# craabreu/EmDee.jl

Hardware: AMD Instinct MI355X
Metric: md_steps_per_sec (higher is better)
Workload: dtype f64

## Files before the change

emdee.jl_amd/csrc/brick.hpp:

```cpp
#pragma once

#include "kernels.hpp"

namespace emdee {

enum BrickMode { BRICK_FORCE = 1, BRICK_STATS = 2, BRICK_STEP = 3 };

#define EMDEE_PLAIN_LOOP _Pragma("clang loop unroll(disable) vectorize(disable) interleave(disable)")

constexpr int EPL = 8;
constexpr int brick_prefetch_blocks(int G, int THREADS) { return (EPL * G) >= 128 ? 1 : ((G == 4 && THREADS >= 1024) ? 5 : 2); }
constexpr int brick_min_stride(int G, int THREADS) { return (brick_prefetch_blocks(G, THREADS) + 1) * EPL * G; }

template <int BX_, int BY_, int BZ_>
struct BrickShape {
    static constexpr int BX = BX_, BY = BY_, BZ = BZ_;
    static constexpr int TX = BX + 2, TY = BY + 2, TZ = BZ + 2;
    static constexpr int NTC = TX * TY * TZ;
    static constexpr int NOC = BX * BY * BZ;
};

struct BrickGrid {
    int nb[3];
    int nbricks;
// ... 1143 lines not shown
    auto slot = [&](unsigned short ent) {
        const int sl = (int)ent >> a.idx_shift;
        int lo = 0, hi = Shape::NTC;
        while (hi - lo > 1) {
            const int mid = (lo + hi) >> 1;
            if (T.off[mid] <= sl) lo = mid; else hi = mid;
        }
        return T.gbeg[lo] + (sl - T.off[lo]);
    };
    for (int o = threadIdx.x; o < n_own; o += THREADS) {
        int ti, p;
        brick_locate(T, o, ti, p);
        if (a.perm[p] >= a.n_owned) continue;
        const int m = min(a.cnt[p], a.stride);
        unsigned short *row = a.nbr + (size_t)p * a.stride;
        const int w = strike_row(keys, bk, a.perm, ex_start, ex_idx, p, m,
                                 [&](int e) -> unsigned short & { return row[row_position<G>((unsigned)e)]; }, slot);
        if (w < 0) continue;
        for (int e = w; e < m; e++) row[row_position<G>((unsigned)e)] = 0;
        a.cnt[p] = w;
    }
}

template <class Shape>
__global__ void k_brick_tile_max(BrickGrid bg, int Mx, int My, int Mz, int px, int py, int pz,
                                 const int *__restrict__ start, int *__restrict__ out) {
    const int b = blockIdx.x * blockDim.x + threadIdx.x;
    int total = 0, own = 0, span3 = 0;
    if (b < bg.nbricks) {
        const int bxi = b % bg.nb[0], byi = (b / bg.nb[0]) % bg.nb[1], bzi = b / (bg.nb[0] * bg.nb[1]);
        const int ox0 = bxi * Shape::BX, oy0 = byi * Shape::BY, oz0 = bzi * Shape::BZ;
        const int ox1 = min(ox0 + Shape::BX, Mx), oy1 = min(oy0 + Shape::BY, My), oz1 = min(oz0 + Shape::BZ, Mz);
        for (int tz = 0; tz < Shape::TZ; tz++)
            for (int ty = 0; ty < Shape::TY; ty++) {
                const int ry = oy0 - 1 + ty, rz = oz0 - 1 + tz;
                int gy = ry, gz = rz;
                if (gy > oy1 || gz > oz1) continue;
                if (gy < 0) { if (!py) continue; gy += My; } else if (gy >= My) { if (!py) continue; gy -= My; }
                if (gz < 0) { if (!pz) continue; gz += Mz; } else if (gz >= Mz) { if (!pz) continue; gz -= Mz; }
                int p1 = 0, p2 = 0;
                for (int tx = 0; tx < Shape::TX; tx++) {
                    const int rx = ox0 - 1 + tx;
                    int gx = rx;
                    bool valid = gx <= ox1;
                    if (gx < 0) { if (!px) valid = false; gx += Mx; } else if (gx >= Mx) { if (!px) valid = false; gx -= Mx; }
                    int pop = 0;
                    if (valid) {
                        const int c = gx + Mx * (gy + My * gz);
                        pop = start[c + 1] - start[c];
                        total += pop;
                        if (rx >= ox0 && rx < ox1 && ry >= oy0 && ry < oy1 && rz >= oz0 && rz < oz1) own += pop;
                    }
                    span3 = max(span3, pop + p1 + p2);
                    p2 = p1; p1 = pop;
                }
            }
    }
#pragma unroll
    for (int off = 1; off < WAVE; off <<= 1) {
        total = max(total, __shfl_xor(total, off));
        own = max(own, __shfl_xor(own, off));
        span3 = max(span3, __shfl_xor(span3, off));
    }
    if ((threadIdx.x & (WAVE - 1)) == 0 && total > 0) {
        atomicMax(&out[0], total);
        atomicMax(&out[1], own);
        atomicMax(&out[2], span3);
    }
}

}
```

emdee.jl_amd/csrc/kernels.hpp:

```cpp
#pragma once

#include <hip/hip_runtime.h>

#include "common.hpp"
#include "lj_pair.hpp"
#include "wave_ops.hpp"

namespace emdee {

template <typename real>
struct Rec;
template <>
struct alignas(32) Rec<double> {
    double x, y, z;
    float hs, te;
};
template <>
struct alignas(16) Rec<float> {
    float x, y, z, hs;
};

struct RelGrid {
    double lo[3], cw[3];
    int M[3];
// ... 217 lines not shown
        } else {
            cell_of[i] = -1;
        }
    }
    int first, len;
    wave_run(c, first, len);
    if (c >= 0 && lane_id() == first) atomicAdd(&count[c], len);
}

static __global__ void k_cell_scatter(int n, const int *__restrict__ cell_of, int one_based, const int *__restrict__ start,
                               int *__restrict__ fill, int *__restrict__ tmp) {
    int i = blockIdx.x * blockDim.x + threadIdx.x;
    const int c = (i < n) ? cell_of[i] - one_based : -1;
    int first, len;
    wave_run(c, first, len);
    int base = 0;
    if (c >= 0 && lane_id() == first) base = start[c] + atomicAdd(&fill[c], len);
    base = __shfl(base, first);
    if (c >= 0) tmp[base + (lane_id() - first)] = i;
}

static __global__ void k_cell_scatter_keyed(int n, const int *__restrict__ cell_of, const int *__restrict__ start,
                                            int *__restrict__ fill, const int *__restrict__ key, int2 *__restrict__ tmp,
                                            const long long *__restrict__ tag = nullptr) {
    int i = blockIdx.x * blockDim.x + threadIdx.x;
    const int c = (i < n) ? cell_of[i] : -1;
    int first, len;
    wave_run(c, first, len);
    int base = 0;
    if (c >= 0 && lane_id() == first) base = start[c] + atomicAdd(&fill[c], len);
    base = __shfl(base, first);
    if (c >= 0) tmp[base + (lane_id() - first)] = make_int2(i, tag ? (int)tag[i] : (key ? key[i] : i));
}
static __global__ void k_cell_rankfix_keyed(int n, const int *__restrict__ cell_of, const int *__restrict__ start,
                                            const int2 *__restrict__ tmp, int *__restrict__ order,
                                            const int *__restrict__ n_dev = nullptr, int ties = 1) {
    int q = blockIdx.x * blockDim.x + threadIdx.x;
    if (n_dev) n = min(n, *n_dev);
    if (q >= n) return;
    const int2 me = tmp[q];
    const int c = cell_of[me.x];
    const int s = start[c], e = start[c + 1];
    int rank = 0;
    if (ties) {
        for (int r = s; r < e; r++) {
            const int2 o = tmp[r];
            rank += (o.y < me.y || (o.y == me.y && o.x < me.x)) ? 1 : 0;
        }
    } else {
        for (int r = s; r < e; r++) rank += (tmp[r].y < me.y) ? 1 : 0;
    }
    order[s + rank] = me.x;
}

static __global__ void k_cell_rankfix(int n, const int *__restrict__ cell_of, int one_based, const int *__restrict__ start,
                               const int *__restrict__ tmp, const int *__restrict__ key, int *__restrict__ order) {
    int q = blockIdx.x * blockDim.x + threadIdx.x;
    if (q >= n) return;
    int i = tmp[q];
    int c = cell_of[i] - one_based;
    int s = start[c], e = start[c + 1];
    int ki = key ? key[i] : i;
    int rank = 0;
    for (int r = s; r < e; r++) {
        int j = tmp[r];
        int kj = key ? key[j] : j;
        rank += (kj < ki) ? 1 : 0;
    }
    order[s + rank] = i;
}

constexpr int SCAN_THREADS = 256;
constexpr int SCAN_ITEMS = 8;
constexpr int SCAN_TILE = SCAN_THREADS * SCAN_ITEMS;

// ... 125 lines not shown
constexpr int IMG_BIAS = 512;
__device__ __forceinline__ int img_pack(int kx, int ky, int kz) {
    return (kx + IMG_BIAS) | ((ky + IMG_BIAS) << 10) | ((kz + IMG_BIAS) << 20);
}
__device__ __forceinline__ void img_unpack(int v, int &kx, int &ky, int &kz) {
    kx = (v & 1023) - IMG_BIAS; ky = ((v >> 10) & 1023) - IMG_BIAS; kz = ((v >> 20) & 1023) - IMG_BIAS;
}
template <typename real>
__device__ __forceinline__ int wrap_into_box(real &p, real lo, real len, int periodic) {
    if (!periodic) return 0;
    const real k = floor((p - lo) / len);
    p -= k * len;
    return (int)k;
}

__device__ __forceinline__ int rel_nearest_image(double &r, double len, int periodic) {
    if (!periodic) return 0;
    const double s = rint(r / len);
    r -= s * len;
    return (int)s;
}

template <typename real>
__global__ void k_gather_user(int n, int n_owned, size_t pitch, GridP<real> g, const int *__restrict__ order,
                              const int *__restrict__ cell_of, const real *__restrict__ pos,
                              const emdee_lj_atom *__restrict__ atoms, const real *__restrict__ vel,
                              const real *__restrict__ inv_mass, Rec<real> *__restrict__ rec, float *__restrict__ te,
                              real *__restrict__ xb, real *__restrict__ v_out, real *__restrict__ im_out,
                              int *__restrict__ perm, int *__restrict__ inv_perm, int *__restrict__ cell_sorted,
                              int *__restrict__ img, int nt = 1, const long long *__restrict__ tag_in = nullptr,
                              long long *__restrict__ tag_out = nullptr, int ncell = 0, int *__restrict__ cstart = nullptr,
                              const int *__restrict__ tstart = nullptr, RelGrid rel_out = RelGrid{}) {
    int p = blockIdx.x * blockDim.x + threadIdx.x;
    if (cstart) for (int c = p; c <= ncell; c += gridDim.x * blockDim.x) cstart[c] = tstart[(size_t)c * nt];
    if (p >= n) return;
    int i = order[p];
    if (tag_out) tag_out[p] = tag_in[i];
    real x = pos[3 * (size_t)i], y = pos[3 * (size_t)i + 1], z = pos[3 * (size_t)i + 2];
    const int kx = wrap_into_box(x, g.lo[0], g.len[0], g.per[0]);
    const int ky = wrap_into_box(y, g.lo[1], g.len[1], g.per[1]);
    const int kz = wrap_into_box(z, g.lo[2], g.len[2], g.per[2]);
    img[p] = img_pack(kx, ky, kz);
    emdee_lj_atom a = atoms[i];
    if (sizeof(real) == 4 && rel_out.on) {
        double ox, oy, oz;
        rel_out.origin(cell_of[i] / nt, ox, oy, oz);
        double rx = (double)x - ox, ry = (double)y - oy, rz = (double)z - oz;
        int jx = kx + rel_nearest_image(rx, (double)g.len[0], g.per[0]), jy = ky + rel_nearest_image(ry, (double)g.len[1], g.per[1]),
            jz = kz + rel_nearest_image(rz, (double)g.len[2], g.per[2]);
        img[p] = img_pack(jx, jy, jz);
        x = (real)rx; y = (real)ry; z = (real)rz;
    }
    store_rec<real>(rec, te, p, x, y, z, a.half_sigma, a.twice_sqrt_eps);
    xb[p] = x; xb[pitch + p] = y; xb[2 * pitch + p] = z;
    bool owned = i < n_owned;
    if (v_out) {
        for (int d = 0; d < 3; d++) v_out[d * pitch + p] = (owned && vel) ? vel[3 * (size_t)i + d] : (real)0;
    }
    if (im_out) im_out[p] = (owned && inv_mass) ? inv_mass[i] : (real)1;
    perm[p] = i;
    inv_perm[i] = p;
    cell_sorted[p] = cell_of[i] / nt;
}

template <typename real, bool EDIT = false>
__global__ void k_gather_sorted(int n, size_t pitch, GridP<real> g, const int *__restrict__ order,
                                const int *__restrict__ cell_of, const Rec<real> *__restrict__ rec_in,
                                const float *__restrict__ te_in, const real *__restrict__ v_in,
                                const real *__restrict__ im_in, const int *__restrict__ perm_in,
                                const int *__restrict__ img_in, Rec<real> *__restrict__ rec, float *__restrict__ te,
                                real *__restrict__ xb, real *__restrict__ v_out, real *__restrict__ im_out,
                                int *__restrict__ perm, int *__restrict__ inv_perm, int *__restrict__ cell_sorted,
                                int *__restrict__ img, int nt = 1, const long long *__restrict__ tag_in = nullptr,
                                long long *__restrict__ tag_out = nullptr, const int *__restrict__ n_dev = nullptr,
                                int *__restrict__ n_out = nullptr, int ncell = 0, int *__restrict__ cstart = nullptr,
                                const int *__restrict__ tstart = nullptr, RelGrid rel_in = RelGrid{}, RelGrid rel_out = RelGrid{}) {
    int p = blockIdx.x * blockDim.x + threadIdx.x;
    if (cstart) for (int c = p; c <= ncell; c += gridDim.x * blockDim.x) cstart[c] = tstart[(size_t)c * nt];
    if (EDIT) {
        n = min(n, *n_dev);
        if (p == 0 && n_out) *n_out = *n_dev;
    }
    if (p >= n) return;
    int o = order[p];
    Rec<real> r = rec_in[o];
    float hs, tev;
    rec_params(rec_in, te_in, o, hs, tev);
    int kx = 0, ky = 0, kz = 0;
    if (!EDIT) img_unpack(img_in[o], kx, ky, kz);
    if (sizeof(real) == 4 && (rel_in.on || rel_out.on)) {
        double ax = (double)r.x, ay = (double)r.y, az = (double)r.z, ox, oy, oz;
        if (rel_in.on) { rel_in.origin(rel_in.cell[o], ox, oy, oz); ax += ox; ay += oy; az += oz; }
        kx += wrap_into_box(ax, (double)g.lo[0], (double)g.len[0], g.per[0]);
        ky += wrap_into_box(ay, (double)g.lo[1], (double)g.len[1], g.per[1]);
        kz += wrap_into_box(az, (double)g.lo[2], (double)g.len[2], g.per[2]);
        if (rel_out.on) {
            rel_out.origin(cell_of[o] / nt, ox, oy, oz); ax -= ox; ay -= oy; az -= oz;
            kx += rel_nearest_image(ax, (double)g.len[0], g.per[0]);
            ky += rel_nearest_image(ay, (double)g.len[1], g.per[1]);
            kz += rel_nearest_image(az, (double)g.len[2], g.per[2]);
        }
        r.x = (real)ax; r.y = (real)ay; r.z = (real)az;
    } else {
        kx += wrap_into_box(r.x, g.lo[0], g.len[0], g.per[0]);
        ky += wrap_into_box(r.y, g.lo[1], g.len[1], g.per[1]);
        kz += wrap_into_box(r.z, g.lo[2], g.len[2], g.per[2]);
    }
    img[p] = img_pack(kx, ky, kz);
    store_rec<real>(rec, te, p, r.x, r.y, r.z, hs, tev);
    xb[p] = r.x; xb[pitch + p] = r.y; xb[2 * pitch + p] = r.z;
    if (v_out) {
        for (int d = 0; d < 3; d++) v_out[d * pitch + p] = v_in[d * pitch + o];
    }
    if (im_out) im_out[p] = im_in[o];
    if (tag_out) tag_out[p] = tag_in[o];
    int i = EDIT ? o : perm_in[o];
    perm[p] = i;
    inv_perm[i] = p;
    cell_sorted[p] = cell_of[o] / nt;
}

template <typename real>
__global__ void k_refresh_positions(int n, size_t pitch, GridP<real> g, const int *__restrict__ perm,
                                    const real *__restrict__ pos, const emdee_lj_atom *__restrict__ atoms,
                                    const real *__restrict__ xb, Rec<real> *__restrict__ rec, float *__restrict__ te) {
    int p = blockIdx.x * blockDim.x + threadIdx.x;
    if (p >= n) return;
    int i = perm[p];
    emdee_lj_atom a = atoms[i];
    const real bx = xb[p], by = xb[pitch + p], bz = xb[2 * pitch + p];
    const real x = bx + min_image(pos[3 * (size_t)i] - bx, g.plen[0], g.pinv[0]);
    const real y = by + min_image(pos[3 * (size_t)i + 1] - by, g.plen[1], g.pinv[1]);
    const real z = bz + min_image(pos[3 * (size_t)i + 2] - bz, g.plen[2], g.pinv[2]);
    store_rec<real>(rec, te, p, x, y, z, a.half_sigma, a.twice_sqrt_eps);
}

template <typename real>
__global__ void k_refresh_check(int n, size_t pitch, GridP<real> g, const int *__restrict__ perm, const real *__restrict__ pos,
                                const emdee_lj_atom *__restrict__ atoms, const real *__restrict__ xb, Rec<real> *__restrict__ rec,
                                float *__restrict__ te, real thr2, int *__restrict__ flags, int typed = 0) {
    int p = blockIdx.x * blockDim.x + threadIdx.x;
    if (p >= n) return;
// ... 946 lines not shown
```

emdee.jl_amd/csrc/nbsys.hpp:

```cpp
#pragma once
#include <cstdio>

#include <algorithm>
#include <cmath>
#include <cstdlib>
#include <type_traits>

#include "brick.hpp"
#include "ewald.hpp"
#include "kernels.hpp"
#include "topology_dev.hpp"
#include "typed.hpp"

namespace emdee {

static inline void refuse_experiment_switches() {
    static const char *const gone[] = {"EMDEE_DEBUG_RC2_SCALE", "EMDEE_TBUILD", "EMDEE_BUILD4", "EMDEE_BUILD_ALG", "EMDEE_BUILD_CHUNKED",
        "EMDEE_BUILD_STRIDED", "EMDEE_NO_BRICK_TABLES", "EMDEE_NO_PREMUL", "EMDEE_BUILD_NEARFAR", "EMDEE_NEAR_DELTA", "EMDEE_FAR_SKIP",
        "EMDEE_PLAN_MAXIMA", "EMDEE_PLAN_SYNC", "EMDEE_STRIDE", "EMDEE_BRICK_VARIANT"};
    for (const char *name : gone)
        EMDEE_REQUIRE(std::getenv(name) == nullptr, EMDEE_ERR_INVALID,
                      "%s is an experiment switch that has been retired with the laboratory (make EXPERIMENTS=1 no longer "
                      "exists): the variant it selected is not built; its measurement is recorded in DESIGN.md, "
                      "\"Product and laboratory\"", name);
// ... 69 lines not shown
    GridP<real> grid{};
    size_t ncell = 0;
    int n_total = 0, n_owned = 0;
    size_t pitch = 0;
    bool with_vel = false, with_mass = false;
    bool sorted = false, has_list = false;
    int stride = 0;
    int64_t builds = 0;
    bool profiling = false;
    KernelTimer timers[T_COUNT];

    int path = PATH_BRICK;
    int variant = 0;
    BrickGrid bgrid{};
    int tile_cap = 0, own_cap = 0, row_block = 1;
    int build_alg = 1;
    bool field16_blocked = false;
    size_t lds_bytes = 0, lds_build_bytes = 0;
    float build_margin = 0.f;

    DevBuf<Rec<real>> rec, rec2;
    DevBuf<float> te, te2;
    DevBuf<real> vel, vel2, frc, en, vir, im, im2, xb, noise;
    DevBuf<int> perm, perm2, inv_perm, cell_of, cell_sorted, cell_sorted2, order, count, fill, nbr, cnt, flags, img, img2;
    DevBuf<int2> tmp2;
    DevBuf<long long> tag, tag2;
    bool use_tags = false;
    size_t cap_hint = 0;
    size_t capacity = 0;
    bool has_ghosts = false;
    int id_space = 0;
    bool id_gaps = false;
    DevBuf<int> cmap;
    bool cmap_valid = false;
    SpeciesTable species{1, {0, 0, 0, 0}};
    int nt = 1;
    int nsub = 1;
    bool subbins_enabled = std::getenv("EMDEE_NO_SUBBINS") == nullptr;
    int tsub = 1;
    bool typed_subbins_enabled = std::getenv("EMDEE_TYPED_SUBBINS") == nullptr || std::atoi(std::getenv("EMDEE_TYPED_SUBBINS")) != 0;
    int digits() const { return nt > 1 ? nt * tsub : nsub; }
    DevBuf<int> bsub;
    bool typed_enabled = std::getenv("EMDEE_NO_TYPED") == nullptr;
    DevBuf<int> cstart;
    DevBuf<unsigned long long> species_tab;
    DevBuf<unsigned short> nbr16;
    DevBuf<int> btab;
// ... 95 lines not shown
            g.per[d] = per[d];
            g.M[d] = M[d];
            cells *= (size_t)M[d];
        }
        g.nd = 1;
        g.one_based = 0;
        grid = g;
        ncell = cells;
    }

    void reserve(int n, bool velocities, bool masses) {
        n_total = n;
        const size_t m = std::max((size_t)n, cap_hint);
        capacity = m;
        pitch = (m + 63) / 64 * 64 + 64;
        with_vel = velocities;
        with_mass = masses;
        rec.ensure(m + 1); rec2.ensure(m + 1);
        if (sizeof(real) == 4) { te.ensure(m + 1); te2.ensure(m + 1); }
        frc.ensure(3 * pitch); en.ensure(pitch); vir.ensure(pitch); xb.ensure(3 * pitch);
        if (velocities) { vel.ensure(3 * pitch); vel2.ensure(3 * pitch); }
        if (masses) { im.ensure(pitch); im2.ensure(pitch); }
        perm.ensure(m + 1); perm2.ensure(m + 1); inv_perm.ensure(m + 1); img.ensure(m + 1); img2.ensure(m + 1);
        cell_of.ensure(m + 1); cell_sorted.ensure(m + 1); cell_sorted2.ensure(m + 1); order.ensure(m + 1); cnt.ensure(m + 1);
        if (use_tags) { tag.ensure(m + 1); tag2.ensure(m + 1); }
        if (flags.ensure(32)) EMDEE_HIP_CHECK(hipMemsetAsync(flags.ptr, 0, 32 * sizeof(int), stream()));
        partial.ensure(3 * RED_MAX_BLOCKS); sums.ensure(8); stats.ensure(4);
    }

    template <class Src, class Spc>
    void bin(Src src, const int *key, Spc spc, int n_items = -1, const long long *tagkey = nullptr, const unsigned char *keep = nullptr) {
        const int n = n_items >= 0 ? n_items : n_total;
        const int dm = digits();
        const size_t nbins = ncell * (size_t)dm;
        count.ensure(nbins + 2); fill.ensure(nbins + 2);
        Zeros zr;
        zr.add(count.ptr, nbins + 1).add(fill.ptr, nbins);
        if (dm > 1) {
            cstart.ensure(ncell + 2);
            if (n == 0) zr.add(cstart.ptr, ncell + 1);
        }
        zr.run(stream());
        if (n == 0) return;
        hipLaunchKernelGGL((k_cell_assign<real, Src, Spc>), dim3(blocks_for(n, 256)), dim3(256), 0, stream(), n, src, grid,
                           cell_of.ptr, count.ptr, spc, dm, keep);
        scanner.run(count.ptr, nbins + 1, stream());
        tmp2.ensure(std::max((size_t)n, capacity) + 1);
        hipLaunchKernelGGL(k_cell_scatter_keyed, dim3(blocks_for(n, 256)), dim3(256), 0, stream(), n, cell_of.ptr, count.ptr,
                           fill.ptr, key, tmp2.ptr, tagkey);
        hipLaunchKernelGGL(k_cell_rankfix_keyed, dim3(blocks_for(n, 256)), dim3(256), 0, stream(), n, cell_of.ptr, count.ptr,
                           tmp2.ptr, order.ptr, keep ? count.ptr + nbins : nullptr, tagkey != nullptr ? 1 : 0);
    }
    int sub_k() const {
        const double cx = len[0] / std::max(1, grid.M[0]);
        const double margin = 16.0 * grid.M[0] * (sizeof(real) == 4 ? 6.0e-8 : 1.2e-16) + 1e-9;
        return std::max(-1, (int)std::floor(4.0 * (1.0 - rlist * (1.0 + margin) / cx)));
    }
    void choose_subbins() {
        nsub = (subbins_enabled && path == PATH_BRICK && nt == 1 && n_total > 0) ? 4 : 1;
        tsub = (subbins_enabled && typed_subbins_enabled && typed_enabled && path == PATH_BRICK && nt == 2 && n_total > 0) ? 4 : 1;
    }
    template <class Src, class Spc>
    void bin_species(Src src, const int *key, Spc spc, int n_items = -1, const long long *tagkey = nullptr, const unsigned char *keep = nullptr) {
        using Sub = XSubBin<real, Src>;
        if (tsub > 1) bin(src, key, SpeciesSub<Spc, Sub>{spc, Sub{src, grid.lo[0], grid.len[0], grid.M[0], grid.per[0], tsub}}, n_items, tagkey, keep);
        else bin(src, key, spc, n_items, tagkey, keep);
    }
    template <class Src>
    void bin_untyped(Src src, const int *key, int n_items = -1, const long long *tagkey = nullptr, const unsigned char *keep = nullptr) {
        if (nsub > 1) bin(src, key, XSubBin<real, Src>{src, grid.lo[0], grid.len[0], grid.M[0], grid.per[0], nsub}, n_items, tagkey, keep);
        else bin(src, key, NoSpecies{}, n_items, tagkey, keep);
    }
    const int *start() const { return digits() > 1 ? cstart.ptr : count.ptr; }
    const int *tstart() const { return count.ptr; }

    void load_user(int n_own, int n_ghost, const real *pos, const real *velocities, const emdee_lj_atom *atoms,
                   const real *inv_mass, const long long *tags_user = nullptr) {
        EMDEE_REQUIRE(n_own >= 0 && n_ghost >= 0, EMDEE_ERR_INVALID, "negative atom count");
        EMDEE_REQUIRE((int64_t)n_own + n_ghost < (int64_t)1 << 31, EMDEE_ERR_INVALID, "too many atoms");
        EMDEE_REQUIRE(n_own + n_ghost == 0 || (pos && atoms), EMDEE_ERR_INVALID, "positions/atoms are NULL");
        Timed t(this, T_REBUILD);
        n_owned = n_own;
        has_ghosts = n_ghost > 0;
        id_space = n_own + n_ghost; id_gaps = false; cmap_valid = false;
        lgv_ids = nullptr;
        use_tags = tags_user != nullptr;
        reserve(n_own + n_ghost, velocities != nullptr || with_vel, inv_mass != nullptr);
        detect_uniform_atoms(atoms);
        configure_grid();
        const int n = n_total;
        const bool rel_next = rel_wanted();
        choose_subbins();
        if (nt > 1) bin_species(UserPos<real>{pos}, nullptr, UserSpecies{species, atoms}, -1, use_tags ? tags_user : nullptr);
        else bin_untyped(UserPos<real>{pos}, nullptr, -1, use_tags ? tags_user : nullptr);
        if (n > 0)
            hipLaunchKernelGGL((k_gather_user<real>), dim3(blocks_for(n, 256)), dim3(256), 0, stream(), n, n_owned, pitch,
                               grid, order.ptr, cell_of.ptr, pos, atoms, velocities, inv_mass, rec.ptr, te.ptr, xb.ptr,
                               with_vel ? vel.ptr : nullptr, with_mass ? im.ptr : nullptr, perm.ptr, inv_perm.ptr,
                               cell_sorted.ptr, img.ptr, digits(), use_tags ? tags_user : nullptr, use_tags ? tag.ptr : nullptr,
                               (int)ncell, digits() > 1 ? cstart.ptr : nullptr, count.ptr, rel_grid_next(rel_next, nullptr));
        rel_commit(rel_next);
        q_valid = false;
        if (has_ghosts)
            hipLaunchKernelGGL((k_copy_ghost_records<real>), dim3(blocks_for(n, 256)), dim3(256), 0, stream(), n, n_owned,
                               perm.ptr, rec.ptr, rec2.ptr);
        sorted = true;
        build_list();
    }

    void resort() {
        EMDEE_REQUIRE(sorted, EMDEE_ERR_STATE, "no state loaded");
        Timed t(this, T_REBUILD);
        const int n = n_total;
        configure_grid();
        choose_subbins();
        const long long *tk = use_tags ? tag.ptr : nullptr;
        const RelGrid rel_in = rel_grid(rel_now, cell_sorted.ptr);
        const bool rel_next = rel_wanted();
        if (nt > 1) bin_species(RecPos<real>{rec.ptr, rel_in}, perm.ptr, RecSpecies<real>{species, rec.ptr, te.ptr}, -1, tk);
        else bin_untyped(RecPos<real>{rec.ptr, rel_in}, perm.ptr, -1, tk);
        if (n > 0)
            hipLaunchKernelGGL((k_gather_sorted<real, false>), dim3(blocks_for(n, 256)), dim3(256), 0, stream(), n, pitch, grid,
                               order.ptr, cell_of.ptr, rec.ptr, te.ptr, with_vel ? vel.ptr : nullptr,
                               with_mass ? im.ptr : nullptr, perm.ptr, img.ptr, rec2.ptr, te2.ptr, xb.ptr,
                               with_vel ? vel2.ptr : nullptr, with_mass ? im2.ptr : nullptr, perm2.ptr, inv_perm.ptr,
                               cell_sorted2.ptr, img2.ptr, digits(), tk, use_tags ? tag2.ptr : nullptr, (const int *)nullptr,
                               (int *)nullptr, (int)ncell, digits() > 1 ? cstart.ptr : nullptr, count.ptr, rel_in,
                               rel_grid_next(rel_next, nullptr));
        swap_sorted_buffers();
        rel_commit(rel_next);
        build_list();
    }
    void check_scaled_box(const double mu[3], double vscale) const {
        for (int d = 0; d < 3; d++)
            EMDEE_REQUIRE(std::isfinite(mu[d]) && mu[d] > 0.0, EMDEE_ERR_INVALID, "scale_box: mu[%d] = %g must be finite and > 0", d, mu[d]);
        EMDEE_REQUIRE(std::isfinite(vscale) && vscale > 0.0, EMDEE_ERR_INVALID, "scale_box: velocity_scale = %g must be finite and > 0", vscale);
        for (int d = 0; d < 3; d++) {
            const double nl = mu[d] * len[d];
            EMDEE_REQUIRE(std::isfinite(nl) && nl > 0.0, EMDEE_ERR_INVALID, "scale_box: the new box length %g along %d is not finite and > 0", nl, d);
            EMDEE_REQUIRE(!per[d] || nl >= 2.0 * rlist, EMDEE_ERR_INVALID, "scale_box: the new periodic box length %g along dimension %d is below "
                          "2 (cutoff + skin) = %g (minimum image)", nl, d, 2.0 * rlist);
        }
    }
    void scale_box(const double mu[3], double vscale) {
        EMDEE_REQUIRE(sorted && with_vel && !has_ghosts, EMDEE_ERR_STATE, "scale_box: needs a loaded state without ghosts");
        check_scaled_box(mu, vscale);
        if (n_total > 0) {
            ScaleBox s{};
            for (int d = 0; d < 3; d++) { s.lo[d] = lo[d]; s.mu[d] = mu[d]; }
            hipLaunchKernelGGL((k_cell_state_scale<real>), dim3(blocks_for(n_total, 256)), dim3(256), 0, stream(), n_total, pitch, rec.ptr,
                               vel.ptr, s, (real)vscale, vscale != 1.0 ? 1 : 0, rel_grid(rel_now, cell_sorted.ptr));
// ... 13 lines not shown

    struct EditWords {
        const int *dev = nullptr;
        int n = 0;
        int32_t *host = nullptr;
    };
    bool in_edit = false, edit_abort = false;
    EditWords edit_extra{};
    int edit_n_plan = 0;
    struct EditSaved { int n_total, n_owned, id_space; bool id_gaps, has_ghosts, has_list; } edit_saved{};
    bool edit_fits(int n_items) const { return sorted && use_tags && with_vel && !with_mass && (size_t)n_items <= capacity; }
    bool edit_extra_read = false;
    bool resort_edit(int n_items, const unsigned char *keep, int own_limit, bool ghosts, int *n_live_dev, EditWords extra) {
        EMDEE_REQUIRE(edit_fits(n_items), EMDEE_ERR_STATE, "resort_edit: the state does not hold %d slots", n_items);
        Timed t(this, T_REBUILD);
        edit_saved = EditSaved{n_total, n_owned, id_space, id_gaps, has_ghosts, has_list};
        configure_grid();
        choose_subbins();
        EMDEE_REQUIRE(!rel_now, EMDEE_ERR_STATE, "resort_edit: cell-relative records (decomposed domains keep absolute ones)");
        if (nt > 1) bin_species(RecPos<real>{rec.ptr, RelGrid{}}, nullptr, RecSpecies<real>{species, rec.ptr, te.ptr}, n_items, tag.ptr, keep);
        else bin_untyped(RecPos<real>{rec.ptr, RelGrid{}}, nullptr, n_items, tag.ptr, keep);
        const size_t nbins = ncell * (size_t)digits();
        hipLaunchKernelGGL((k_gather_sorted<real, true>), dim3(blocks_for(n_items, 256)), dim3(256), 0, stream(), n_items, pitch, grid,
                           order.ptr, cell_of.ptr, rec.ptr, te.ptr, vel.ptr, (const real *)nullptr, perm.ptr, img.ptr, rec2.ptr, te2.ptr,
                           xb.ptr, vel2.ptr, (real *)nullptr, perm2.ptr, inv_perm.ptr, cell_sorted2.ptr, img2.ptr, digits(), tag.ptr,
                           tag2.ptr, count.ptr + nbins, n_live_dev, (int)ncell, digits() > 1 ? cstart.ptr : nullptr, count.ptr);
        swap_sorted_buffers();
        edit_n_plan = n_total;
        n_total = n_items;
        n_owned = own_limit;
        has_ghosts = ghosts;
        id_space = n_items; id_gaps = true; cmap_valid = false;
        in_edit = true; edit_abort = false; edit_extra = extra; edit_extra_read = false;
        struct Leave { bool &f; ~Leave() { f = false; } } leave{in_edit};
        if (path == PATH_BRICK && plan_valid && edit_saved.n_total > 0) build_list();
        else edit_abort = true;
        if (edit_abort && !edit_extra_read && extra.n > 0) read_back_words(ctx, stream(), extra.dev, extra.n, extra.host);
        return !edit_abort;
    }
    void commit_edit(int n_live) {
        EMDEE_REQUIRE(n_live >= 0 && n_live <= n_total, EMDEE_ERR_STATE, "resort_edit: %d atoms in %d slots", n_live, n_total);
        n_total = n_live;
        if (has_ghosts && n_total > 0)
            hipLaunchKernelGGL((k_copy_ghost_records<real>), dim3(blocks_for(n_total, 256)), dim3(256), 0, stream(), n_total, n_owned,
                               perm.ptr, rec.ptr, rec2.ptr);
    }
    void rollback_edit() {
        swap_sorted_buffers();
        n_total = edit_saved.n_total; n_owned = edit_saved.n_owned; id_space = edit_saved.id_space;
// ... 147 lines not shown
            bgrid.nbricks = bgrid.nb[0] * bgrid.nb[1] * bgrid.nb[2];
            bgrid.per_xcd = (bgrid.nbricks + NXCD - 1) / NXCD;
            const int B[3] = {S::BX, S::BY, S::BZ};
            bgrid.ib_count = 1;
            for (int d = 0; d < 3; d++) {
                int lo_b = 0, n_b = bgrid.nb[d];
                if (!grid.per[d]) {
                    lo_b = 1;
                    int hi_b = 1;
                    while (hi_b < bgrid.nb[d] && (hi_b + 1) * B[d] < grid.M[d] - 1) hi_b++;
                    n_b = std::max(0, hi_b - lo_b);
                }
                bgrid.ib_lo[d] = lo_b; bgrid.ib_n[d] = n_b;
                bgrid.ib_count *= n_b;
            }
            bgrid.ib_per_xcd = (bgrid.ib_count + NXCD - 1) / NXCD;
            bgrid.bb_z = (bgrid.nb[2] - bgrid.ib_n[2]) * bgrid.nb[0] * bgrid.nb[1];
            bgrid.bb_y = bgrid.ib_n[2] * (bgrid.nb[1] - bgrid.ib_n[1]) * bgrid.nb[0];
            bgrid.bb_count = bgrid.nbricks - bgrid.ib_count;
            bgrid.bb_per_xcd = (bgrid.bb_count + NXCD - 1) / NXCD;
            row_block = EPL * V::G;
        });
    }
    void launch_tile_max(bool with_build_words = false) {
        with_brick_variant(variant, [&](auto v) {
            using S = typename decltype(v)::Shape;
            if (with_build_words) Zeros().add(flags.ptr, 9).run(stream());
            else Zeros().add(flags.ptr + 6, 3).run(stream());
            hipLaunchKernelGGL((k_brick_tile_max<S>), dim3(blocks_for(bgrid.nbricks, 256)), dim3(256), 0, stream(), bgrid,
                               grid.M[0], grid.M[1], grid.M[2], grid.per[0], grid.per[1], grid.per[2], start(),
                               flags.ptr + 6);
        });
    }
    static int with_headroom(int v) { return (v + v / 32 + 8 + 15) / 16 * 16; }
    bool plan_sizes(int max_tile, int max_own, int max_span3) {
        bool ok = true;
        with_brick_variant(variant, [&](auto v) {
            using V = decltype(v);
            using S = typename V::Shape;
            tile_cap = std::max(64, with_headroom(max_tile + 1));
            if (max_tile + 1 <= SOA_SLOTS) tile_cap = std::min(tile_cap, SOA_SLOTS);
            own_cap = std::max(64, with_headroom(max_own));
            {
                const int exact = std::max(64, (max_tile + 1 + 15) / 16 * 16), st = stride > 0 ? stride : 128;
                constexpr size_t USABLE = 150000;
                auto per_cu = [&](int tc) {
                    const size_t b = brick_build_lds_bytes<S, V::THREADS>(tc, own_cap, st, V::GB, nsub),
                                 f = brick_force_lds_bytes<real, S, V::THREADS>(tc, own_cap, has_charges());
                    return (int)(USABLE / std::max<size_t>(b, 1)) * 16 + (int)(USABLE / std::max<size_t>(f, 1));
                };
                while (tile_cap > exact && per_cu(tile_cap) < per_cu(exact)) tile_cap -= 16;
            }
// ... 140 lines not shown
    bool typed_blocked = false;
    bool typed_stride = false;

    void build_list() {
        const int n = n_total;
        if (stride == 0) {
            double vol = len[0] * len[1] * len[2];
            double expect = n > 0 ? (4.0 / 3.0) * M_PI * rlist * rlist * rlist * (double)n / vol : 0.0;
            stride = (int)((expect * 1.15 + 8.0) / 16.0 + 1.0) * 16;
            typed_stride = false;
        }
        btab_valid = false;
        const int np = in_edit ? edit_n_plan : n;
        bool kept = plan_valid && path == PATH_BRICK && n > 0 && plan_M[0] == grid.M[0] &&
                    plan_M[1] == grid.M[1] && plan_M[2] == grid.M[2] && plan_n <= np + np / 8 && np <= plan_n + plan_n / 8 &&
                    plan_uniform == uniform_atoms && plan_nt == nt && plan_charged == has_charges();
        if (kept) {
            plan_geometry();
            launch_tile_max(true);
            brick_active = true;
        } else {
            make_plan();
        }
        const size_t rows = std::max<size_t>((size_t)std::max(n, 1), cap_hint ? capacity : 0);
        for (int attempt = 0; attempt < 6; attempt++) {
            EMDEE_REQUIRE((double)n * stride < 1.7e10, EMDEE_ERR_OVERFLOW, "neighbour list would exceed 64 GiB");
            if (in_edit && !brick_active) { edit_abort = true; return; }
            if (!(kept && attempt == 0)) Zeros().add(flags.ptr, 5).run(stream());
            if (brick_active) {
                nbr16.ensure(rows * stride);
                with_brick_variant(variant, [&](auto v) {
                    using V = decltype(v);
                    if constexpr (typed_variant<V>()) {
                        if (typed_active) {
                            constexpr int TT = 256;
                            using BT = TypedTables<typename V::Shape, TT>;
                            static_assert(BT::row_ints() == TypedTables<typename V::Shape, V::THREADS>::row_ints(), "table row layout");
                            btab.ensure((size_t)bgrid.nbricks * BT::row_ints());
                            BrickArgs<real> ta = brick_args();
                            ta.btab = btab.ptr;
                            if (tsub > 1) {
                                bsub.ensure((size_t)bgrid.nbricks * BT::NTT + 4);
                                ta.nsub = tsub; ta.bsub = bsub.ptr;
                            }
                            hipLaunchKernelGGL((k_typed_tables<real, typename V::Shape, TT>), dim3(bgrid.per_xcd * NXCD), dim3(TT),
                                               BT::bytes(0), stream(), ta);
// ... 375 lines not shown
        if (has_post()) return false;
        if (phase != 2 && !noise_ready) prepare_noise(dt);
        {
            Timed t(this, phase == 2 ? T_STEP_BOUNDARY : T_STEP);
            step_c = c; step_dt = dt;
            force_phase = phase;
            step_guard = guard; step_trigger = trigger;
            with_brick_variant(variant, [&](auto v) { launch_brick_kernel<decltype(v), BRICK_STEP, 1>(); });
            step_guard = nullptr; step_trigger = nullptr;
        }
        if (phase != 1 && lgv_on) lgv_step++;
        if (phase != 1) {
            if (carry_ghosts && has_ghosts)
                hipLaunchKernelGGL((k_copy_ghost_records<real>), dim3(blocks_for(n_total, 256)), dim3(256), 0, stream(),
                                   n_total, n_owned, perm.ptr, rec.ptr, rec2.ptr);
            swap_step_buffers();
        }
        return true;
    }
    void swap_step_buffers() { rec.swap(rec2); vel.swap(vel2); }

    static constexpr int RUN_AHEAD = 4;
    int run_ahead = RUN_AHEAD;
    int *step_trigger = nullptr;
    const int *step_guard = nullptr;
    int fused_steps_run_ahead(double c, double dt, int want, bool *stale) {
        EMDEE_REQUIRE(has_list && sorted && with_vel, EMDEE_ERR_STATE, "no state loaded");
        *stale = false;
        if (!brick_active || n_total == 0 || has_ghosts || has_post()) return 0;
        const int B = std::max(1, std::min(want, run_ahead));
        int *words = flags.ptr + 9;
        EMDEE_HIP_CHECK(hipMemsetAsync(words, 0, B * sizeof(int), stream()));
        step_c = c; step_dt = dt; force_phase = 0;
        for (int i = 0; i < B; i++) {
            prepare_noise(dt);
            if (lgv_on) lgv_step++;
            Timed t(this, T_STEP);
            step_trigger = words + i;
            step_guard = i ? words + i - 1 : nullptr;
            with_brick_variant(variant, [&](auto v) { launch_brick_kernel<decltype(v), BRICK_STEP, 1>(); });
            swap_step_buffers();
        }
        step_trigger = nullptr; step_guard = nullptr;
        read_back_words(ctx, stream(), words, B, ctx->host_flags + 9);
        int ran = B;
        for (int i = 0; i < B; i++)
            if (ctx->host_flags[9 + i]) { ran = i + 1; *stale = true; break; }
        if ((B - ran) & 1) swap_step_buffers();
        if (lgv_on) lgv_step -= (unsigned long long)(B - ran);
        if (profiling) timers[T_STEP].dropped += B - ran;
        return ran;
    }

    real *out_f = nullptr, *out_e = nullptr, *out_w = nullptr;
    real *out_vt = nullptr;
// ... 197 lines not shown
```

Baseline: 538.0.

## Fuse rank-fix into gather kernels and parallelize tile-max over sub-lanes

Drops the separate rank-fix kernel and the order buffer: the gather kernels now compute each atom's sorted slot directly from the scattered (index,key) pairs. The cstart copy and the clearing of the flag words move into the scatter kernel, so the later memset launches can be skipped through new 'already clear' flags. The tile-max kernel now spreads each brick's rows over 16 lanes with 1024-thread blocks and a shared-memory reduction. The aim is fewer launches and memsets per rebuild, at the cost of extra state flags that must stay in sync.

```diff
diff --git a/emdee.jl_amd/csrc/brick.hpp b/emdee.jl_amd/csrc/brick.hpp
--- a/emdee.jl_amd/csrc/brick.hpp
+++ b/emdee.jl_amd/csrc/brick.hpp
@@ -1189,51 +1189,69 @@
     }
 }
 
+constexpr int TILE_MAX_LANES = 16, TILE_MAX_THREADS = 1024;
 template <class Shape>
-__global__ void k_brick_tile_max(BrickGrid bg, int Mx, int My, int Mz, int px, int py, int pz,
-                                 const int *__restrict__ start, int *__restrict__ out) {
-    const int b = blockIdx.x * blockDim.x + threadIdx.x;
+__global__ __launch_bounds__(TILE_MAX_THREADS) void k_brick_tile_max(BrickGrid bg, int Mx, int My, int Mz, int px, int py, int pz,
+                                                                     const int *__restrict__ start, int *__restrict__ out) {
+    constexpr int ROWS = Shape::TY * Shape::TZ, NW = TILE_MAX_THREADS / WAVE;
+    static_assert(WAVE % TILE_MAX_LANES == 0, "the lanes of a brick share a wavefront");
+    __shared__ int red[3][NW];
+    const int t = blockIdx.x * TILE_MAX_THREADS + threadIdx.x;
+    const int b = t / TILE_MAX_LANES, sub = t % TILE_MAX_LANES;
     int total = 0, own = 0, span3 = 0;
     if (b < bg.nbricks) {
         const int bxi = b % bg.nb[0], byi = (b / bg.nb[0]) % bg.nb[1], bzi = b / (bg.nb[0] * bg.nb[1]);
         const int ox0 = bxi * Shape::BX, oy0 = byi * Shape::BY, oz0 = bzi * Shape::BZ;
         const int ox1 = min(ox0 + Shape::BX, Mx), oy1 = min(oy0 + Shape::BY, My), oz1 = min(oz0 + Shape::BZ, Mz);
-        for (int tz = 0; tz < Shape::TZ; tz++)
-            for (int ty = 0; ty < Shape::TY; ty++) {
-                const int ry = oy0 - 1 + ty, rz = oz0 - 1 + tz;
-                int gy = ry, gz = rz;
-                if (gy > oy1 || gz > oz1) continue;
-                if (gy < 0) { if (!py) continue; gy += My; } else if (gy >= My) { if (!py) continue; gy -= My; }
-                if (gz < 0) { if (!pz) continue; gz += Mz; } else if (gz >= Mz) { if (!pz) continue; gz -= Mz; }
-                int p1 = 0, p2 = 0;
-                for (int tx = 0; tx < Shape::TX; tx++) {
-                    const int rx = ox0 - 1 + tx;
-                    int gx = rx;
-                    bool valid = gx <= ox1;
-                    if (gx < 0) { if (!px) valid = false; gx += Mx; } else if (gx >= Mx) { if (!px) valid = false; gx -= Mx; }
-                    int pop = 0;
-                    if (valid) {
-                        const int c = gx + Mx * (gy + My * gz);
-                        pop = start[c + 1] - start[c];
-                        total += pop;
-                        if (rx >= ox0 && rx < ox1 && ry >= oy0 && ry < oy1 && rz >= oz0 && rz < oz1) own += pop;
-                    }
-                    span3 = max(span3, pop + p1 + p2);
-                    p2 = p1; p1 = pop;
-                }
-            }
-    }
-#pragma unroll
-    for (int off = 1; off < WAVE; off <<= 1) {
+        for (int row = sub; row < ROWS; row += TILE_MAX_LANES) {
+            const int ty = row % Shape::TY, tz = row / Shape::TY;
+            const int ry = oy0 - 1 + ty, rz = oz0 - 1 + tz;
+            int gy = ry, gz = rz;
+            if (gy > oy1 || gz > oz1) continue;
+            if (gy < 0) { if (!py) continue; gy += My; } else if (gy >= My) { if (!py) continue; gy -= My; }
+            if (gz < 0) { if (!pz) continue; gz += Mz; } else if (gz >= Mz) { if (!pz) continue; gz -= Mz; }
+            int p1 = 0, p2 = 0;
+            for (int tx = 0; tx < Shape::TX; tx++) {
+                const int rx = ox0 - 1 + tx;
+                int gx = rx;
+                bool valid = gx <= ox1;
+                if (gx < 0) { if (!px) valid = false; gx += Mx; } else if (gx >= Mx) { if (!px) valid = false; gx -= Mx; }
+                int pop = 0;
+                if (valid) {
+                    const int c = gx + Mx * (gy + My * gz);
+                    pop = start[c + 1] - start[c];
+                    total += pop;
+                    if (rx >= ox0 && rx < ox1 && ry >= oy0 && ry < oy1 && rz >= oz0 && rz < oz1) own += pop;
+                }
+                span3 = max(span3, pop + p1 + p2);
+                p2 = p1; p1 = pop;
+            }
+        }
+    }
+#pragma unroll
+    for (int off = 1; off < TILE_MAX_LANES; off <<= 1) {
+        total += __shfl_xor(total, off);
+        own += __shfl_xor(own, off);
+        span3 = max(span3, __shfl_xor(span3, off));
+    }
+#pragma unroll
+    for (int off = TILE_MAX_LANES; off < WAVE; off <<= 1) {
         total = max(total, __shfl_xor(total, off));
         own = max(own, __shfl_xor(own, off));
         span3 = max(span3, __shfl_xor(span3, off));
     }
-    if ((threadIdx.x & (WAVE - 1)) == 0 && total > 0) {
-        atomicMax(&out[0], total);
-        atomicMax(&out[1], own);
-        atomicMax(&out[2], span3);
-    }
-}
-
-}
+    const int lane = threadIdx.x & (WAVE - 1), wv = threadIdx.x / WAVE;
+    if (lane == 0) { red[0][wv] = total; red[1][wv] = own; red[2][wv] = span3; }
+    __syncthreads();
+    if (threadIdx.x < 3) {
+        int m = 0;
+#pragma unroll
+        for (int w = 0; w < NW; w++) m = max(m, red[threadIdx.x][w]);
+        int any = 0;
+#pragma unroll
+        for (int w = 0; w < NW; w++) any = max(any, red[0][w]);
+        if (any > 0) atomicMax(&out[threadIdx.x], m);
+    }
+}
+
+}
diff --git a/emdee.jl_amd/csrc/kernels.hpp b/emdee.jl_amd/csrc/kernels.hpp
--- a/emdee.jl_amd/csrc/kernels.hpp
+++ b/emdee.jl_amd/csrc/kernels.hpp
@@ -263,8 +263,12 @@
 
 static __global__ void k_cell_scatter_keyed(int n, const int *__restrict__ cell_of, const int *__restrict__ start,
                                             int *__restrict__ fill, const int *__restrict__ key, int2 *__restrict__ tmp,
-                                            const long long *__restrict__ tag = nullptr) {
+                                            const long long *__restrict__ tag = nullptr, int ncell = 0, int nt = 1,
+                                            int *__restrict__ cstart = nullptr, int *__restrict__ zero_words = nullptr,
+                                            int zero_n = 0) {
     int i = blockIdx.x * blockDim.x + threadIdx.x;
+    if (cstart) for (int c = i; c <= ncell; c += gridDim.x * blockDim.x) cstart[c] = start[(size_t)c * nt];
+    if (i < zero_n) zero_words[i] = 0;
     const int c = (i < n) ? cell_of[i] : -1;
     int first, len;
     wave_run(c, first, len);
@@ -273,14 +277,7 @@
     base = __shfl(base, first);
     if (c >= 0) tmp[base + (lane_id() - first)] = make_int2(i, tag ? (int)tag[i] : (key ? key[i] : i));
 }
-static __global__ void k_cell_rankfix_keyed(int n, const int *__restrict__ cell_of, const int *__restrict__ start,
-                                            const int2 *__restrict__ tmp, int *__restrict__ order,
-                                            const int *__restrict__ n_dev = nullptr, int ties = 1) {
-    int q = blockIdx.x * blockDim.x + threadIdx.x;
-    if (n_dev) n = min(n, *n_dev);
-    if (q >= n) return;
-    const int2 me = tmp[q];
-    const int c = cell_of[me.x];
+__device__ __forceinline__ int ranked_slot(const int2 *__restrict__ tmp, const int *__restrict__ start, int c, int2 me, int ties) {
     const int s = start[c], e = start[c + 1];
     int rank = 0;
     if (ties) {
@@ -291,7 +288,7 @@
     } else {
         for (int r = s; r < e; r++) rank += (tmp[r].y < me.y) ? 1 : 0;
     }
-    order[s + rank] = me.x;
+    return s + rank;
 }
 
 static __global__ void k_cell_rankfix(int n, const int *__restrict__ cell_of, int one_based, const int *__restrict__ start,
@@ -463,19 +460,20 @@
 }
 
 template <typename real>
-__global__ void k_gather_user(int n, int n_owned, size_t pitch, GridP<real> g, const int *__restrict__ order,
+__global__ void k_gather_user(int n, int n_owned, size_t pitch, GridP<real> g, const int2 *__restrict__ tmp, int ties,
                               const int *__restrict__ cell_of, const real *__restrict__ pos,
                               const emdee_lj_atom *__restrict__ atoms, const real *__restrict__ vel,
                               const real *__restrict__ inv_mass, Rec<real> *__restrict__ rec, float *__restrict__ te,
                               real *__restrict__ xb, real *__restrict__ v_out, real *__restrict__ im_out,
                               int *__restrict__ perm, int *__restrict__ inv_perm, int *__restrict__ cell_sorted,
                               int *__restrict__ img, int nt = 1, const long long *__restrict__ tag_in = nullptr,
-                              long long *__restrict__ tag_out = nullptr, int ncell = 0, int *__restrict__ cstart = nullptr,
-                              const int *__restrict__ tstart = nullptr, RelGrid rel_out = RelGrid{}) {
-    int p = blockIdx.x * blockDim.x + threadIdx.x;
-    if (cstart) for (int c = p; c <= ncell; c += gridDim.x * blockDim.x) cstart[c] = tstart[(size_t)c * nt];
-    if (p >= n) return;
-    int i = order[p];
+                              long long *__restrict__ tag_out = nullptr, const int *__restrict__ tstart = nullptr,
+                              RelGrid rel_out = RelGrid{}) {
+    const int q = blockIdx.x * blockDim.x + threadIdx.x;
+    if (q >= n) return;
+    const int2 me = tmp[q];
+    const int i = me.x, bin = cell_of[i];
+    const int p = ranked_slot(tmp, tstart, bin, me, ties);
     if (tag_out) tag_out[p] = tag_in[i];
     real x = pos[3 * (size_t)i], y = pos[3 * (size_t)i + 1], z = pos[3 * (size_t)i + 2];
     const int kx = wrap_into_box(x, g.lo[0], g.len[0], g.per[0]);
@@ -485,7 +483,7 @@
     emdee_lj_atom a = atoms[i];
     if (sizeof(real) == 4 && rel_out.on) {
         double ox, oy, oz;
-        rel_out.origin(cell_of[i] / nt, ox, oy, oz);
+        rel_out.origin(bin / nt, ox, oy, oz);
         double rx = (double)x - ox, ry = (double)y - oy, rz = (double)z - oz;
         int jx = kx + rel_nearest_image(rx, (double)g.len[0], g.per[0]), jy = ky + rel_nearest_image(ry, (double)g.len[1], g.per[1]),
             jz = kz + rel_nearest_image(rz, (double)g.len[2], g.per[2]);
@@ -501,11 +499,11 @@
     if (im_out) im_out[p] = (owned && inv_mass) ? inv_mass[i] : (real)1;
     perm[p] = i;
     inv_perm[i] = p;
-    cell_sorted[p] = cell_of[i] / nt;
+    cell_sorted[p] = bin / nt;
 }
 
 template <typename real, bool EDIT = false>
-__global__ void k_gather_sorted(int n, size_t pitch, GridP<real> g, const int *__restrict__ order,
+__global__ void k_gather_sorted(int n, size_t pitch, GridP<real> g, const int2 *__restrict__ tmp, int ties,
                                 const int *__restrict__ cell_of, const Rec<real> *__restrict__ rec_in,
                                 const float *__restrict__ te_in, const real *__restrict__ v_in,
                                 const real *__restrict__ im_in, const int *__restrict__ perm_in,
@@ -514,16 +512,17 @@
                                 int *__restrict__ perm, int *__restrict__ inv_perm, int *__restrict__ cell_sorted,
                                 int *__restrict__ img, int nt = 1, const long long *__restrict__ tag_in = nullptr,
                                 long long *__restrict__ tag_out = nullptr, const int *__restrict__ n_dev = nullptr,
-                                int *__restrict__ n_out = nullptr, int ncell = 0, int *__restrict__ cstart = nullptr,
-                                const int *__restrict__ tstart = nullptr, RelGrid rel_in = RelGrid{}, RelGrid rel_out = RelGrid{}) {
-    int p = blockIdx.x * blockDim.x + threadIdx.x;
-    if (cstart) for (int c = p; c <= ncell; c += gridDim.x * blockDim.x) cstart[c] = tstart[(size_t)c * nt];
+                                int *__restrict__ n_out = nullptr, const int *__restrict__ tstart = nullptr,
+                                RelGrid rel_in = RelGrid{}, RelGrid rel_out = RelGrid{}) {
+    const int q = blockIdx.x * blockDim.x + threadIdx.x;
     if (EDIT) {
         n = min(n, *n_dev);
-        if (p == 0 && n_out) *n_out = *n_dev;
-    }
-    if (p >= n) return;
-    int o = order[p];
+        if (q == 0 && n_out) *n_out = *n_dev;
+    }
+    if (q >= n) return;
+    const int2 me = tmp[q];
+    const int o = me.x, bin = cell_of[o];
+    const int p = ranked_slot(tmp, tstart, bin, me, ties);
     Rec<real> r = rec_in[o];
     float hs, tev;
     rec_params(rec_in, te_in, o, hs, tev);
@@ -536,7 +535,7 @@
         ky += wrap_into_box(ay, (double)g.lo[1], (double)g.len[1], g.per[1]);
         kz += wrap_into_box(az, (double)g.lo[2], (double)g.len[2], g.per[2]);
         if (rel_out.on) {
-            rel_out.origin(cell_of[o] / nt, ox, oy, oz); ax -= ox; ay -= oy; az -= oz;
+            rel_out.origin(bin / nt, ox, oy, oz); ax -= ox; ay -= oy; az -= oz;
             kx += rel_nearest_image(ax, (double)g.len[0], g.per[0]);
             ky += rel_nearest_image(ay, (double)g.len[1], g.per[1]);
             kz += rel_nearest_image(az, (double)g.len[2], g.per[2]);
@@ -558,7 +557,7 @@
     int i = EDIT ? o : perm_in[o];
     perm[p] = i;
     inv_perm[i] = p;
-    cell_sorted[p] = cell_of[o] / nt;
+    cell_sorted[p] = bin / nt;
 }
 
 template <typename real>
diff --git a/emdee.jl_amd/csrc/nbsys.hpp b/emdee.jl_amd/csrc/nbsys.hpp
--- a/emdee.jl_amd/csrc/nbsys.hpp
+++ b/emdee.jl_amd/csrc/nbsys.hpp
@@ -115,7 +115,7 @@
     DevBuf<Rec<real>> rec, rec2;
     DevBuf<float> te, te2;
     DevBuf<real> vel, vel2, frc, en, vir, im, im2, xb, noise;
-    DevBuf<int> perm, perm2, inv_perm, cell_of, cell_sorted, cell_sorted2, order, count, fill, nbr, cnt, flags, img, img2;
+    DevBuf<int> perm, perm2, inv_perm, cell_of, cell_sorted, cell_sorted2, count, fill, nbr, cnt, flags, img, img2;
     DevBuf<int2> tmp2;
     DevBuf<long long> tag, tag2;
     bool use_tags = false;
@@ -257,7 +257,7 @@
         if (velocities) { vel.ensure(3 * pitch); vel2.ensure(3 * pitch); }
         if (masses) { im.ensure(pitch); im2.ensure(pitch); }
         perm.ensure(m + 1); perm2.ensure(m + 1); inv_perm.ensure(m + 1); img.ensure(m + 1); img2.ensure(m + 1);
-        cell_of.ensure(m + 1); cell_sorted.ensure(m + 1); cell_sorted2.ensure(m + 1); order.ensure(m + 1); cnt.ensure(m + 1);
+        cell_of.ensure(m + 1); cell_sorted.ensure(m + 1); cell_sorted2.ensure(m + 1); cnt.ensure(m + 1);
         if (use_tags) { tag.ensure(m + 1); tag2.ensure(m + 1); }
         if (flags.ensure(32)) EMDEE_HIP_CHECK(hipMemsetAsync(flags.ptr, 0, 32 * sizeof(int), stream()));
         partial.ensure(3 * RED_MAX_BLOCKS); sums.ensure(8); stats.ensure(4);
@@ -276,16 +276,19 @@
             if (n == 0) zr.add(cstart.ptr, ncell + 1);
         }
         zr.run(stream());
+        build_words_clear = false;
         if (n == 0) return;
         hipLaunchKernelGGL((k_cell_assign<real, Src, Spc>), dim3(blocks_for(n, 256)), dim3(256), 0, stream(), n, src, grid,
                            cell_of.ptr, count.ptr, spc, dm, keep);
         scanner.run(count.ptr, nbins + 1, stream());
         tmp2.ensure(std::max((size_t)n, capacity) + 1);
         hipLaunchKernelGGL(k_cell_scatter_keyed, dim3(blocks_for(n, 256)), dim3(256), 0, stream(), n, cell_of.ptr, count.ptr,
-                           fill.ptr, key, tmp2.ptr, tagkey);
-        hipLaunchKernelGGL(k_cell_rankfix_keyed, dim3(blocks_for(n, 256)), dim3(256), 0, stream(), n, cell_of.ptr, count.ptr,
-                           tmp2.ptr, order.ptr, keep ? count.ptr + nbins : nullptr, tagkey != nullptr ? 1 : 0);
-    }
+                           fill.ptr, key, tmp2.ptr, tagkey, (int)ncell, dm, dm > 1 ? cstart.ptr : nullptr, flags.ptr,
+                           BUILD_WORDS + RUN_AHEAD);
+        build_words_clear = true; step_words_clear = true;
+        bin_ties = tagkey != nullptr ? 1 : 0;
+    }
+    int bin_ties = 0;
     int sub_k() const {
         const double cx = len[0] / std::max(1, grid.M[0]);
         const double margin = 16.0 * grid.M[0] * (sizeof(real) == 4 ? 6.0e-8 : 1.2e-16) + 1e-9;
@@ -330,10 +333,10 @@
         else bin_untyped(UserPos<real>{pos}, nullptr, -1, use_tags ? tags_user : nullptr);
         if (n > 0)
             hipLaunchKernelGGL((k_gather_user<real>), dim3(blocks_for(n, 256)), dim3(256), 0, stream(), n, n_owned, pitch,
-                               grid, order.ptr, cell_of.ptr, pos, atoms, velocities, inv_mass, rec.ptr, te.ptr, xb.ptr,
+                               grid, tmp2.ptr, bin_ties, cell_of.ptr, pos, atoms, velocities, inv_mass, rec.ptr, te.ptr, xb.ptr,
                                with_vel ? vel.ptr : nullptr, with_mass ? im.ptr : nullptr, perm.ptr, inv_perm.ptr,
                                cell_sorted.ptr, img.ptr, digits(), use_tags ? tags_user : nullptr, use_tags ? tag.ptr : nullptr,
-                               (int)ncell, digits() > 1 ? cstart.ptr : nullptr, count.ptr, rel_grid_next(rel_next, nullptr));
+                               count.ptr, rel_grid_next(rel_next, nullptr));
         rel_commit(rel_next);
         q_valid = false;
         if (has_ghosts)
@@ -356,12 +359,11 @@
         else bin_untyped(RecPos<real>{rec.ptr, rel_in}, perm.ptr, -1, tk);
         if (n > 0)
             hipLaunchKernelGGL((k_gather_sorted<real, false>), dim3(blocks_for(n, 256)), dim3(256), 0, stream(), n, pitch, grid,
-                               order.ptr, cell_of.ptr, rec.ptr, te.ptr, with_vel ? vel.ptr : nullptr,
+                               tmp2.ptr, bin_ties, cell_of.ptr, rec.ptr, te.ptr, with_vel ? vel.ptr : nullptr,
                                with_mass ? im.ptr : nullptr, perm.ptr, img.ptr, rec2.ptr, te2.ptr, xb.ptr,
                                with_vel ? vel2.ptr : nullptr, with_mass ? im2.ptr : nullptr, perm2.ptr, inv_perm.ptr,
                                cell_sorted2.ptr, img2.ptr, digits(), tk, use_tags ? tag2.ptr : nullptr, (const int *)nullptr,
-                               (int *)nullptr, (int)ncell, digits() > 1 ? cstart.ptr : nullptr, count.ptr, rel_in,
-                               rel_grid_next(rel_next, nullptr));
+                               (int *)nullptr, count.ptr, rel_in, rel_grid_next(rel_next, nullptr));
         swap_sorted_buffers();
         rel_commit(rel_next);
         build_list();
@@ -421,9 +423,9 @@
         else bin_untyped(RecPos<real>{rec.ptr, RelGrid{}}, nullptr, n_items, tag.ptr, keep);
         const size_t nbins = ncell * (size_t)digits();
         hipLaunchKernelGGL((k_gather_sorted<real, true>), dim3(blocks_for(n_items, 256)), dim3(256), 0, stream(), n_items, pitch, grid,
-                           order.ptr, cell_of.ptr, rec.ptr, te.ptr, vel.ptr, (const real *)nullptr, perm.ptr, img.ptr, rec2.ptr, te2.ptr,
+                           tmp2.ptr, bin_ties, cell_of.ptr, rec.ptr, te.ptr, vel.ptr, (const real *)nullptr, perm.ptr, img.ptr, rec2.ptr, te2.ptr,
                            xb.ptr, vel2.ptr, (real *)nullptr, perm2.ptr, inv_perm.ptr, cell_sorted2.ptr, img2.ptr, digits(), tag.ptr,
-                           tag2.ptr, count.ptr + nbins, n_live_dev, (int)ncell, digits() > 1 ? cstart.ptr : nullptr, count.ptr);
+                           tag2.ptr, count.ptr + nbins, n_live_dev, count.ptr);
         swap_sorted_buffers();
         edit_n_plan = n_total;
         n_total = n_items;
@@ -617,12 +619,18 @@
             row_block = EPL * V::G;
         });
     }
+    static constexpr int BUILD_WORDS = 9;
+    bool build_words_clear = false;
     void launch_tile_max(bool with_build_words = false) {
+        const hipStream_t s = stream();
         with_brick_variant(variant, [&](auto v) {
             using S = typename decltype(v)::Shape;
-            if (with_build_words) Zeros().add(flags.ptr, 9).run(stream());
-            else Zeros().add(flags.ptr + 6, 3).run(stream());
-            hipLaunchKernelGGL((k_brick_tile_max<S>), dim3(blocks_for(bgrid.nbricks, 256)), dim3(256), 0, stream(), bgrid,
+            if (with_build_words && build_words_clear) {}
+            else if (with_build_words) Zeros().add(flags.ptr, BUILD_WORDS).run(s);
+            else Zeros().add(flags.ptr + 6, 3).run(s);
+            build_words_clear = false;
+            hipLaunchKernelGGL((k_brick_tile_max<S>), dim3(blocks_for((size_t)bgrid.nbricks * TILE_MAX_LANES, TILE_MAX_THREADS)),
+                               dim3(TILE_MAX_THREADS), 0, s, bgrid,
                                grid.M[0], grid.M[1], grid.M[2], grid.per[0], grid.per[1], grid.per[2], start(),
                                flags.ptr + 6);
         });
@@ -809,6 +817,7 @@
         } else {
             make_plan();
         }
+        build_words_clear = false;
         const size_t rows = std::max<size_t>((size_t)std::max(n, 1), cap_hint ? capacity : 0);
         for (int attempt = 0; attempt < 6; attempt++) {
             EMDEE_REQUIRE((double)n * stride < 1.7e10, EMDEE_ERR_OVERFLOW, "neighbour list would exceed 64 GiB");
@@ -1230,6 +1239,7 @@
 
     static constexpr int RUN_AHEAD = 4;
     int run_ahead = RUN_AHEAD;
+    bool step_words_clear = false;
     int *step_trigger = nullptr;
     const int *step_guard = nullptr;
     int fused_steps_run_ahead(double c, double dt, int want, bool *stale) {
@@ -1237,8 +1247,9 @@
         *stale = false;
         if (!brick_active || n_total == 0 || has_ghosts || has_post()) return 0;
         const int B = std::max(1, std::min(want, run_ahead));
-        int *words = flags.ptr + 9;
-        EMDEE_HIP_CHECK(hipMemsetAsync(words, 0, B * sizeof(int), stream()));
+        int *words = flags.ptr + BUILD_WORDS;
+        if (!step_words_clear) EMDEE_HIP_CHECK(hipMemsetAsync(words, 0, B * sizeof(int), stream()));
+        step_words_clear = false;
         step_c = c; step_dt = dt; force_phase = 0;
         for (int i = 0; i < B; i++) {
             prepare_noise(dt);
```

Result: no change. 541.3 (median of 6 runs) (+0.6%).
